# tjysdsg/speech-recognition

Measured on AMD Instinct MI355X. Metric: frame-state loglik/s + utterances/s Viterbi decode, higher is better.
Workload: dtype f64; 1 GPU; configs[1]: 10-digit HMM, 5 states/digit, 8-mix GMM, 39-dim, 10000 utterances/GPU (999364 frames on rank 0), isolated-word decode; states=50, mixtures=8, dim=39, parallelism=utterance-sharded x1, batches_in_flight=2, process_group=single

## Files before the change

speech-recognition_amd/csrc/gh_loglik_mfma.hip:

```cpp
#include "gh_internal.h"
#include "gh_wave.h"

namespace {

typedef double v4d __attribute__((ext_vector_type(4)));
typedef float v4f __attribute__((ext_vector_type(4)));

struct gh_loglik_blk { int64_t n0; int32_t nrows, t0, t1, pad; };

template <typename T> struct Acc;
template <> struct Acc<double> {
    typedef v4d type;
    static __device__ __forceinline__ v4d mfma(double a, double b, v4d c) {
        return __builtin_amdgcn_mfma_f64_16x16x4f64(a, b, c, 0, 0, 0);
    }
};
template <> struct Acc<float> {
    typedef v4f type;
    static __device__ __forceinline__ v4f mfma(float a, float b, v4f c) {
        return __builtin_amdgcn_mfma_f32_16x16x4f32(a, b, c, 0, 0, 0);
    }
};

struct Fp64Tables {
    double exp2[128];
    double inv[128];
    double nlog[128];
};

template <typename T> struct Dom;
template <> struct Dom<double> {
    static constexpr double inv_k = 1.0 / GH_LSE_SCALE64, off = GH_LSE_OFF64, off_test = GH_LSE_OFF64 * 0.1;
};
template <> struct Dom<float> {
    static constexpr float inv_k = (float)(1.0 / GH_LSE_SCALE32), off = GH_LSE_OFF32, off_test = GH_LSE_OFF32 * 0.1f;
};

struct LseK {
    double e3 = 2.6466421444330968834e-08;
    double l4 = -46.166241308446829036, l3 = 61.554988411262438714;
    double l2 = -92.332482616893658071, l1 = 184.66496523378731614;
    __device__ __forceinline__ void pin() {
        asm volatile("" : "+v"(e3), "+v"(l4), "+v"(l3), "+v"(l2), "+v"(l1));
    }
};

__device__ __forceinline__ double logs(double s, const double* __restrict__ tab, const LseK& k) {
    const double* __restrict__ inv = tab + 128;
    const double* __restrict__ nlog = tab + 256;
    const double m = __builtin_amdgcn_frexp_mant(s);
    const int e = __builtin_amdgcn_frexp_exp(s);
    const int j = (__double2hiint(m) >> 13) & 127;
    const double rho = fma(m, inv[j], -1.0);
    double p = fma(rho, 36.932993046757463228, k.l4);
    p = fma(p, rho, k.l3);
    p = fma(p, rho, k.l2);
    p = fma(p, rho, k.l1);
    return fma(p, rho, nlog[j]) + (double)(e << 7);
}
__device__ __forceinline__ float logs(float s, const double*, const LseK&) { return __builtin_amdgcn_logf(s); }

template <int W> __device__ __forceinline__ void swap_rows(unsigned v, unsigned& a, unsigned& b) {
    if (W == 16) {
        auto r = __builtin_amdgcn_permlane16_swap(v, v, false, false);
        a = r[0]; b = r[1];
    } else {
        auto r = __builtin_amdgcn_permlane32_swap(v, v, false, false);
        a = r[0]; b = r[1];
    }
}
template <int W> __device__ __forceinline__ void pair_of(float v, float& a, float& b) {
    unsigned x, y;
    swap_rows<W>(__float_as_uint(v), x, y);
    a = __uint_as_float(x); b = __uint_as_float(y);
}
template <int W> __device__ __forceinline__ void pair_of(double v, double& a, double& b) {
    unsigned xl, yl, xh, yh;
    swap_rows<W>((unsigned)__double2loint(v), xl, yl);
    swap_rows<W>((unsigned)__double2hiint(v), xh, yh);
    a = __hiloint2double((int)xh, (int)xl); b = __hiloint2double((int)yh, (int)yl);
}
template <typename T, int W> __device__ __forceinline__ T pair_max(T v) { T a, b; pair_of<W>(v, a, b); return vmax(a, b); }
template <typename T, int W> __device__ __forceinline__ T pair_sum(T v) { T a, b; pair_of<W>(v, a, b); return a + b; }
__device__ __forceinline__ void pair_split(float v0, float v1, float& a, float& b) {
    auto r = __builtin_amdgcn_permlane16_swap(__float_as_uint(v0), __float_as_uint(v1), false, false);
    a = __uint_as_float(r[0]); b = __uint_as_float(r[1]);
}
__device__ __forceinline__ void pair_split(double v0, double v1, double& a, double& b) {
    auto lo = __builtin_amdgcn_permlane16_swap((unsigned)__double2loint(v0), (unsigned)__double2loint(v1), false, false);
    auto hi = __builtin_amdgcn_permlane16_swap((unsigned)__double2hiint(v0), (unsigned)__double2hiint(v1), false, false);
    a = __hiloint2double((int)hi[0], (int)lo[0]); b = __hiloint2double((int)hi[1], (int)lo[1]);
}
template <typename T> __device__ __forceinline__ T pair_sum_split(T v0, T v1) { T a, b; pair_split(v0, v1, a, b); return a + b; }
template <typename T> __device__ __forceinline__ T pair_max_split(T v0, T v1) { T a, b; pair_split(v0, v1, a, b); return vmax(a, b); }

template <typename T> __device__ __forceinline__ T nll_of(T mx, T sm, const double* tab, T inf_below, const LseK& k) {
    const T v = (mx + logs(sm, tab, k)) * -Dom<T>::inv_k;
    return (mx < inf_below) ? T(INFINITY) : v;
}

template <typename T, typename V> __device__ __forceinline__ T lane_max(const V& a) { return vmax(vmax(a[0], a[1]), vmax(a[2], a[3])); }
template <typename T, typename V> __device__ __forceinline__ T lane_terms(const V& a, T m, const double* tab, const LseK& k) {
    return (exp2s(a[0] - m, tab, k.e3) + exp2s(a[1] - m, tab, k.e3)) + (exp2s(a[2] - m, tab, k.e3) + exp2s(a[3] - m, tab, k.e3));
}
template <typename T, typename V>
__device__ __forceinline__ void tile_lse(const V& a, int width, T& mx, T& sm, const double* tab, const LseK& k) {
    T m = lane_max<T, V>(a);
    if (width >= 2) m = pair_max<T, 16>(m);
    if (width >= 4) m = pair_max<T, 32>(m);
    T e = lane_terms<T, V>(a, m, tab, k);
    if (width >= 2) e = pair_sum<T, 16>(e);
    if (width >= 4) e = pair_sum<T, 32>(e);
    mx = m;
    sm = e;
}

__device__ __forceinline__ float exp2s_fe(double y) { return __builtin_amdgcn_exp2f((float)y * 0.0078125f); }
template <int W> __device__ __forceinline__ float pair_sum_f(float v) { float a, b; pair_of<W>(v, a, b); return a + b; }
template <typename V>
__device__ __forceinline__ void tile_lse_fe(const V& a, int width, double& mx, float& sm) {
    double m = vmax(vmax(a[0], a[1]), vmax(a[2], a[3]));
    if (width >= 2) m = pair_max<double, 16>(m);
    if (width >= 4) m = pair_max<double, 32>(m);
    float e = (exp2s_fe(a[0] - m) + exp2s_fe(a[1] - m)) + (exp2s_fe(a[2] - m) + exp2s_fe(a[3] - m));
    if (width >= 2) e = pair_sum_f<16>(e);
    if (width >= 4) e = pair_sum_f<32>(e);
    mx = m;
    sm = e;
}
__device__ __forceinline__ double nll_of_fe(double mx, float sm, double inf_below) {
    const double v = (mx + (double)(128.0f * __builtin_amdgcn_logf(sm))) * -Dom<double>::inv_k;
    return (mx < inf_below) ? (double)INFINITY : v;
}

template <typename T> using global_ptr = const T __attribute__((address_space(1)))*;
template <typename T> __device__ __forceinline__ global_ptr<T> uniform_ptr(const T* p) {
    uint32_t lo = (uint32_t)reinterpret_cast<uintptr_t>(p), hi = (uint32_t)(reinterpret_cast<uintptr_t>(p) >> 32);
    asm("" : "+s"(lo), "+s"(hi));
    return (global_ptr<T>)reinterpret_cast<const T*>(((uintptr_t)hi << 32) | lo);
}

template <typename T, typename V, int MP, bool FE = false>
__device__ __forceinline__ void tile_epilogue(const V& acc0, const V& acc1, int t, int f, int q, int S, int RS,
                                              int chunk_s0, int tiles_per_state, T* lds, T* dummy,
                                              const double* tab, T (&run_mx)[2], T (&run_sm)[2], T inf_below, const LseK& k) {
    T* orow0 = lds + f * RS - chunk_s0;
    T* orow1 = orow0 + 16 * RS;
    if (MP == 1) {
        const int s = 16 * t + 4 * q;
#pragma unroll
        for (int c = 0; c < 2; ++c) {
            const V& acc = c ? acc1 : acc0;
            T* orow = c ? orow1 : orow0;
#pragma unroll
            for (int r = 0; r < 4; ++r)
                *((s + r < S) ? orow + s + r : dummy) = (acc[r] < inf_below) ? T(INFINITY) : acc[r] * -Dom<T>::inv_k;
        }
    } else if (MP == 2) {
        const int s = 8 * t + 2 * q;
#pragma unroll
        for (int c = 0; c < 2; ++c) {
            const V& acc = c ? acc1 : acc0;
            T* orow = c ? orow1 : orow0;
#pragma unroll
            for (int h = 0; h < 2; ++h) {
                const T x0 = acc[2 * h], x1 = acc[2 * h + 1];
                const T m = vmax(x0, x1);
                const T e = exp2s(x0 - m, tab, k.e3) + exp2s(x1 - m, tab, k.e3);
                *((s + h < S) ? orow + s + h : dummy) = nll_of<T>(m, e, tab, inf_below, k);
            }
        }
#ifdef GH_MF_NOEPI
    } else if (MP <= 16) {
        const int s = (16 / MP) * t + q / (MP / 4);
        *(((q & (MP / 4 - 1)) == 0 && s < S) ? orow0 + s : dummy) = -((acc0[0] + acc0[1]) + (acc0[2] + acc0[3]));
        *(((q & (MP / 4 - 1)) == 0 && s < S) ? orow1 + s : dummy) = -((acc1[0] + acc1[1]) + (acc1[2] + acc1[3]));
#endif
    } else if (FE && MP == 4) {
        if constexpr (FE) {
            double mx; float sm;
            const int s = 4 * t + q;
            tile_lse_fe<V>(acc0, 1, mx, sm);
            *((s < S) ? orow0 + s : dummy) = nll_of_fe(mx, sm, inf_below);
            tile_lse_fe<V>(acc1, 1, mx, sm);
            *((s < S) ? orow1 + s : dummy) = nll_of_fe(mx, sm, inf_below);
        }
    } else if (FE && MP <= 16) {
        if constexpr (FE) {
            constexpr int width = MP / 4;
            double mx0, mx1; float sm0, sm1;
            tile_lse_fe<V>(acc0, width, mx0, sm0);
            tile_lse_fe<V>(acc1, width, mx1, sm1);
            const bool odd = q & 1;
            const int s = (16 / MP) * t + q / width;
            const double v = nll_of_fe(odd ? mx1 : mx0, odd ? sm1 : sm0, inf_below);
            *(((q & (width - 1)) < 2 && s < S) ? (odd ? orow1 : orow0) + s : dummy) = v;
        }
    } else if (FE) {
        if constexpr (FE) {
            const bool last = (t + 1) % tiles_per_state == 0;
            const int s = t / tiles_per_state;
#pragma unroll
            for (int c = 0; c < 2; ++c) {
                double mx; float smf;
                tile_lse_fe<V>(c ? acc1 : acc0, 4, mx, smf);
                const double d = run_mx[c] - mx;
                const float e = exp2s_fe((d > 0.0) ? -d : d);
                const float rs = (float)run_sm[c];
                run_sm[c] = (double)((d > 0.0) ? fmaf(smf, e, rs) : fmaf(rs, e, smf));
                run_mx[c] = (d > 0.0) ? run_mx[c] : mx;
            }
            const bool odd = q & 1;
            const double v = nll_of_fe(odd ? run_mx[1] : run_mx[0], (float)(odd ? run_sm[1] : run_sm[0]), inf_below);
            *((last && q < 2 && s < S) ? (odd ? orow1 : orow0) + s : dummy) = v;
#pragma unroll
            for (int c = 0; c < 2; ++c) {
                run_mx[c] = last ? Dom<T>::off : run_mx[c];
                run_sm[c] = last ? T(0) : run_sm[c];
            }
        }
    } else if (MP == 4) {
        T mx, sm;
        const int s = 4 * t + q;
        tile_lse<T, V>(acc0, 1, mx, sm, tab, k);
        *((s < S) ? orow0 + s : dummy) = nll_of<T>(mx, sm, tab, inf_below, k);
        tile_lse<T, V>(acc1, 1, mx, sm, tab, k);
        *((s < S) ? orow1 + s : dummy) = nll_of<T>(mx, sm, tab, inf_below, k);
    } else if (MP <= 16) {
        constexpr int width = MP / 4;
        T mxs = pair_max_split(lane_max<T, V>(acc0), lane_max<T, V>(acc1));
        if (width >= 4) mxs = pair_max<T, 32>(mxs);
        T mx0, mx1;
        pair_of<16>(mxs, mx0, mx1);
        T sm = pair_sum_split(lane_terms<T, V>(acc0, mx0, tab, k), lane_terms<T, V>(acc1, mx1, tab, k));
        if (width >= 4) sm = pair_sum<T, 32>(sm);
        const bool odd = q & 1;
        const int s = (16 / MP) * t + q / width;
        const T v = nll_of<T>(mxs, sm, tab, inf_below, k);
        *(((q & (width - 1)) < 2 && s < S) ? (odd ? orow1 : orow0) + s : dummy) = v;
    } else {
        const bool last = (t + 1) % tiles_per_state == 0;
        const int s = t / tiles_per_state;
#pragma unroll
        for (int c = 0; c < 2; ++c) {
            T mx, sm;
            tile_lse<T, V>(c ? acc1 : acc0, 4, mx, sm, tab, k);
            const T d = run_mx[c] - mx;
            const T e = exp2s((d > T(0)) ? -d : d, tab, k.e3);
            run_sm[c] = (d > T(0)) ? fma(sm, e, run_sm[c]) : fma(run_sm[c], e, sm);
            run_mx[c] = (d > T(0)) ? run_mx[c] : mx;
        }
        const bool odd = q & 1;
        const T v = nll_of<T>(odd ? run_mx[1] : run_mx[0], odd ? run_sm[1] : run_sm[0], tab, inf_below, k);
        *((last && q < 2 && s < S) ? (odd ? orow1 : orow0) + s : dummy) = v;
#pragma unroll
        for (int c = 0; c < 2; ++c) {
            run_mx[c] = last ? Dom<T>::off : run_mx[c];
            run_sm[c] = last ? T(0) : run_sm[c];
        }
    }
}

#ifndef GH_MF_SGB
#define GH_MF_SGB 0
#endif
template <typename T, int KS, int MP, bool MULTI, bool FE = false>
__global__ __launch_bounds__(64, (sizeof(T) == 4 ? 3 : 1)) void loglik_mfma_kernel(const T* __restrict__ X, int64_t N, int D,
                                                         const T* __restrict__ Apk, const T* __restrict__ Cpk,
                                                         int n_tiles, int S, int M_pad, int chunk_tiles,
                                                         const double* __restrict__ tables, int tab_off,
                                                         T* __restrict__ out, int bpw,
                                                         const gh_loglik_blk* __restrict__ blk_tab, int64_t n_blk,
                                                         const T* __restrict__ cen, T inf_below) {
    typedef typename Acc<T>::type V;
#ifndef GH_MF_RING32
#define GH_MF_RING32 2
#endif
#ifndef GH_MF_RING64
#define GH_MF_RING64 1
#endif
    constexpr int R = KS / (sizeof(T) == 4 ? GH_MF_RING32 : GH_MF_RING64);
    extern __shared__ __attribute__((aligned(16))) unsigned char smem_raw[];
    T* lds = reinterpret_cast<T*>(smem_raw);
    const int lane = threadIdx.x;
    const int f = lane & 15, q = lane >> 4;
    const int64_t n_blocks = (N + 31) / 32;
    int64_t n0 = (int64_t)blockIdx.x * (MULTI ? bpw : 1) * 32;
#ifdef GH_MF_TIMING
    long long tk[5], tw[2];
    tk[0] = clock64(); tw[0] = wall_clock64();
#endif
    int nrows = 0;
    const bool subset = MULTI && blk_tab != nullptr;
    const int64_t kb0 = (int64_t)blockIdx.x * (MULTI ? bpw : 1);
    int t_lo = subset ? blk_tab[kb0].t0 : 0, t_hi = n_tiles, nxt_t0 = 0;
    double* tab = reinterpret_cast<double*>(smem_raw + tab_off);
    if (sizeof(T) == 8 && MP != 1) {
        double tr[6];
#pragma unroll
        for (int it = 0; it < 6; ++it) tr[it] = tables[lane + 64 * it];
#pragma unroll
        for (int it = 0; it < 6; ++it) tab[lane + 64 * it] = tr[it];
    }
    auto stage_frames = [&]() {
        const int nelem = nrows * D;
        const T* src = X + n0 * D;
        T xr[KS];
#pragma unroll
        for (int it = 0; it < KS; ++it) {
            const int i = lane + 64 * it;
            xr[it] = (i < nelem) ? src[i] : T(0);
        }
#pragma unroll
        for (int it = 0; it < KS; ++it) {
            const int i = lane + 64 * it;
            if (i < nelem) lds[i] = xr[it];
        }
        __syncthreads();
    };
    constexpr int KQ = KS / 2;
    T b[2][KS];
    T cen_r[KQ];
#pragma unroll
    for (int j = 0; j < KQ; ++j) cen_r[j] = (sizeof(T) == 4 && cen) ? cen[4 * j + q] : T(0);
    auto build_b = [&]() {
#pragma unroll
        for (int c = 0; c < 2; ++c) {
            const int row = 16 * c + f;
#pragma unroll
            for (int j = 0; j < KQ; ++j) {
                const int d = 4 * j + q;
                T v = (row < nrows && d < D) ? lds[row * D + d] : T(0);
                if (sizeof(T) == 4) v = (row < nrows && d < D) ? v - cen_r[j] : T(0);
                b[c][j] = v * v;
                b[c][KQ + j] = v;
            }
        }
        __syncthreads();
    };

    const int tiles_per_state = (MP <= 16) ? 1 : M_pad / 16;
    const int SC = (MP <= 16) ? chunk_tiles * (16 / (MP <= 16 ? MP : 16)) : chunk_tiles / tiles_per_state;
    const int RS = (S <= SC) ? S : SC;
    T* dummy = lds + 32 * RS + lane;
    T run_mx[2] = {Dom<T>::off, Dom<T>::off}, run_sm[2] = {T(0), T(0)};
    LseK lse_k;
    if (sizeof(T) == 8 && !MULTI && !FE && MP != 1) lse_k.pin();
    int chunk_s0 = 0;
    int subset_cnt = 0;

    T ring[R];
#pragma unroll
    for (int j = 0; j < R; ++j) ring[j] = Apk[((int64_t)t_lo * KS + j) * 64 + lane];
    V c_a, c_b, p0, p1;
#pragma unroll
    for (int r = 0; r < 4; ++r) c_a[r] = Cpk[t_lo * 16 + 4 * q + r];

    auto mfma_tile = [&](int t, V& acc0, V& acc1, const V& c_use, V& c_load) {
        const int tn = (!MULTI || t + 1 < t_hi) ? t + 1 : nxt_t0;
        const global_ptr<T> cp = uniform_ptr(Cpk + (unsigned)(tn * 16));
#pragma unroll
        for (int r = 0; r < 4; ++r) c_load[r] = cp[4 * q + r];
        constexpr int WIN = 4096 / (64 * (int)sizeof(T)), NW = (KS + WIN - 1) / WIN;
        global_ptr<T> a_cur[NW], a_nxt[NW];
#pragma unroll
        for (int w = 0; w < NW; ++w) {
            a_cur[w] = uniform_ptr(Apk + (unsigned)(t * (KS * 64) + w * (WIN * 64)));
            a_nxt[w] = uniform_ptr(Apk + (unsigned)(tn * (KS * 64) + w * (WIN * 64)));
        }
#pragma unroll
        for (int ks = 0; ks < KS; ++ks) {
            const T a = ring[ks % R];
#ifdef GH_MF_NOMFMA
            if (ks == 0) { acc0 = c_use; acc1 = c_use; }
            if (ks % 8 == 0) { acc0[ks % 4] += a * b[0][ks]; acc1[ks % 4] += a * b[1][ks]; }
            else asm volatile("" :: "v"(a));
#else
            acc0 = Acc<T>::mfma(a, b[0][ks], ks == 0 ? c_use : acc0);
            acc1 = Acc<T>::mfma(a, b[1][ks], ks == 0 ? c_use : acc1);
#endif
#ifndef GH_MF_NOLOAD
            ring[ks % R] = (ks + R < KS) ? a_cur[(ks + R) / WIN][((ks + R) % WIN) * 64 + lane]
                                         : a_nxt[(ks + R - KS) / WIN][((ks + R - KS) % WIN) * 64 + lane];
#endif
        }
    };
    auto flush = [&]() {
        const int cnt = subset ? subset_cnt : ((chunk_s0 + SC < S) ? chunk_s0 + SC : S) - chunk_s0;
        __syncthreads();
        if (cnt == S && !subset) {
            typedef T V16 __attribute__((ext_vector_type(16 / sizeof(T))));
            constexpr int VE = 16 / sizeof(T);
            T* dst = out + n0 * S;
            const int total = nrows * S;
            const int nvec = total / VE;
#pragma unroll 4
            for (int i = lane; i < nvec; i += 64)
                reinterpret_cast<V16*>(dst)[i] = reinterpret_cast<const V16*>(lds)[i];
            for (int i = nvec * VE + lane; i < total; i += 64) dst[i] = lds[i];
        } else if (cnt > 0) {
            const int total = nrows * cnt;
            for (int i = lane; i < total; i += 64) {
                const int r = i / cnt, j = i - r * cnt;
                out[(n0 + r) * S + chunk_s0 + j] = lds[r * RS + j];
            }
        }
        __syncthreads();
        chunk_s0 += SC;
    };

    const int nb = MULTI ? bpw : 1;
    int64_t staged_n0 = -1;
    for (int ib = 0; ib < nb; ++ib, n0 += 32) {
        if (subset) {
            const int64_t k = kb0 + ib;
            if (k >= n_blk) break;
            const gh_loglik_blk bd = blk_tab[k];
            n0 = bd.n0; nrows = bd.nrows; t_lo = bd.t0; t_hi = bd.t1;
            nxt_t0 = (ib + 1 < nb && k + 1 < n_blk) ? blk_tab[k + 1].t0 : bd.t0;
        } else {
            if (MULTI && n0 >= N) break;
            nrows = (int)((N - n0 < 32) ? (N - n0) : 32);
        }
        if (!(subset && ib > 0 && n0 == staged_n0)) {
#ifdef GH_MF_PRIO
            __builtin_amdgcn_s_setprio(3);
#endif
            stage_frames();
            build_b();
#ifdef GH_MF_PRIO
            __builtin_amdgcn_s_setprio(0);
#endif
            staged_n0 = n0;
        }
        chunk_s0 = (MP <= 16) ? t_lo * (16 / (MP <= 16 ? MP : 16)) : t_lo / tiles_per_state;
        if (subset) {
            const int s_end = (MP <= 16) ? t_hi * (16 / (MP <= 16 ? MP : 16)) : t_hi / tiles_per_state;
            subset_cnt = ((s_end < S) ? s_end : S) - chunk_s0;
        }
#ifdef GH_MF_TIMING
        tk[1] = clock64();
        tk[2] = tk[1];
#endif
        auto epi = [&](const V& e0, const V& e1, int t) {
            tile_epilogue<T, V, MP, FE>(e0, e1, t, f, q, S, RS, chunk_s0, tiles_per_state, lds, dummy, tab, run_mx, run_sm, inf_below, lse_k);
#pragma unroll
            for (int i = 0; i < (GH_MF_SGB ? 2 * KS : 0); ++i) {
                __builtin_amdgcn_sched_group_barrier(0x008, 1, 0);
                __builtin_amdgcn_sched_group_barrier(0x002, sizeof(T) == 8 ? 5 : 3, 0);
            }
            if (!subset && (t + 1) % chunk_tiles == 0 && t + 1 < n_tiles) flush();
        };
        V r0, r1;
        const int tb = MULTI ? t_lo : 0, te = MULTI ? t_hi : n_tiles;
        mfma_tile(tb, p0, p1, c_a, c_b);
        if (sizeof(T) == 8) {
            int t = tb + 1;
            for (; t + 1 < te; t += 2) {
                mfma_tile(t, r0, r1, c_b, c_a);
                epi(p0, p1, t - 1);
                mfma_tile(t + 1, p0, p1, c_a, c_b);
                epi(r0, r1, t);
            }
            if (t < te) {
                mfma_tile(t, r0, r1, c_b, c_a);
                epi(p0, p1, t - 1);
                epi(r0, r1, t);
            } else {
                epi(p0, p1, te - 1);
                if (MULTI) c_a = c_b;
            }
        } else {
            for (int t = tb + 1; t < te; ++t) {
                mfma_tile(t, r0, r1, c_b, c_a);
                epi(p0, p1, t - 1);
                p0 = r0;
                p1 = r1;
                c_b = c_a;
            }
            epi(p0, p1, te - 1);
            if (MULTI) c_a = c_b;
        }
#ifdef GH_MF_TIMING
        tk[3] = clock64();
#endif
        flush();
#ifdef GH_MF_TIMING
        tk[4] = clock64(); tw[1] = wall_clock64();
        if (lane == 0 && S >= 8) {
            T* o = out + n0 * S;
            for (int i = 0; i < 5; ++i) o[i] = (T)(double)(tk[i] - tk[0]);
            o[5] = (T)(double)(tw[0] & 0xffffffffffll); o[6] = (T)(double)(tw[1] - tw[0]);
            o[7] = (T)(double)__builtin_amdgcn_s_getreg((4 << 0) | (0 << 6) | (31 << 11));
        }
#endif
    }
}

static void chunk_shape(const gh_gmm* g, int* chunk_tiles_out, int* SC_out) {
    const int M_pad = g->M_pad, n_tiles = g->n_tiles, S = g->S;
    int chunk_tiles;
    if (M_pad <= 16) {
        const int spt = 16 / M_pad;
        chunk_tiles = (S <= 64) ? n_tiles : std::max(1, 64 / spt);
    } else {
        const int tps = M_pad / 16;
        chunk_tiles = (S <= 64) ? n_tiles : 64 * tps;
    }
    *chunk_tiles_out = chunk_tiles;
    *SC_out = (M_pad <= 16) ? chunk_tiles * (16 / M_pad) : chunk_tiles / (M_pad / 16);
}

static int build_blk_table(const gh_gmm* g, const gh_batch* b, int SC, const int32_t* st_lo, const int32_t* st_hi,
                           const int64_t* rng_off, std::vector<gh_loglik_blk>& tabv, int* max_tiles_out,
                           const uint8_t* include = nullptr) {
    const int M_pad = g->M_pad, S = g->S;
    int max_tiles = 1;
    std::vector<std::pair<int, int>> runs;
    for (int64_t u = 0; u < b->U; ++u) {
        if (include && !include[u]) continue;
        runs.clear();
        const int64_t r0 = rng_off ? rng_off[u] : u, r1 = rng_off ? rng_off[u + 1] : u + 1;
        for (int64_t r = r0; r < r1; ++r) {
            const int lo = st_lo[r], hi = st_hi[r];
            if (lo < 0 || hi > S || lo >= hi) { gh_set_error("gh_loglik_subset: utterance %lld has state range [%d, %d)", (long long)u, lo, hi); return GH_ERR_INVALID; }
            int t0, t1;
            if (M_pad <= 16) { const int spt = 16 / M_pad; t0 = lo / spt; t1 = (hi + spt - 1) / spt; }
            else { const int tps = M_pad / 16; t0 = lo * tps; t1 = hi * tps; }
            runs.push_back({t0, t1});
        }
        std::sort(runs.begin(), runs.end());
        size_t w = 0;
        for (size_t i = 0; i < runs.size(); ++i) {
            if (w > 0 && runs[i].first <= runs[w - 1].second) runs[w - 1].second = std::max(runs[w - 1].second, runs[i].second);
            else runs[w++] = runs[i];
        }
        runs.resize(w);
        for (const auto& tr : runs) {
            const int t0 = tr.first, t1 = tr.second;
            const int span = (M_pad <= 16) ? (t1 - t0) * (16 / M_pad) : (t1 - t0) / (M_pad / 16);
            if (span > SC) return 1;
            max_tiles = std::max(max_tiles, t1 - t0);
        }
        for (int64_t f = b->offsets[u]; f < b->offsets[u + 1]; f += 32)
            for (const auto& tr : runs)
                tabv.push_back(gh_loglik_blk{f, (int32_t)std::min<int64_t>(32, b->offsets[u + 1] - f), tr.first, tr.second, 0});
    }
    *max_tiles_out = max_tiles;
    return GH_OK;
}

template <typename T>
int launch_mfma_t(gh_ctx* ctx, const gh_gmm* g, gh_batch* b, const T* Apk, const T* Cpk, const int32_t* st_lo,
                  const int32_t* st_hi, const T* cen, const int64_t* rng_off, const gh_loglik_plan* plan) {
    const int64_t N = b->N;
    if (N == 0) return GH_OK;
    const int KS = g->KP / 2;
    const int M_pad = g->M_pad, n_tiles = g->n_tiles, S = g->S;
    int chunk_tiles, SC;
    chunk_shape(g, &chunk_tiles, &SC);
    size_t lds = ((size_t)32 * std::max(std::min(SC, S), g->D) + 64) * sizeof(T);
    lds = (lds + 15) & ~size_t(15);
    const int tab_off = (int)lds;
    if (sizeof(T) == 8 && M_pad != 1) lds += 384 * sizeof(double);
    const double* tables = ctx->d_fp64_tables;
    const T inf_below = (ctx->compat & 1) ? (T)(-745.1332191019412 * (sizeof(T) == 8 ? GH_LSE_SCALE64 : GH_LSE_SCALE32)) : Dom<T>::off_test;
    gh_loglik_blk* d_blk = nullptr;
    int64_t n_blk = 0;
    int max_tiles = n_tiles;
    if (plan) {
        d_blk = static_cast<gh_loglik_blk*>(plan->d_blk);
        n_blk = plan->n_blk;
        max_tiles = plan->max_tiles;
        if (n_blk == 0) return GH_OK;
    } else if (st_lo) {
        std::vector<gh_loglik_blk> tabv;
        int rc = build_blk_table(g, b, SC, st_lo, st_hi, rng_off, tabv, &max_tiles);
        if (rc) return rc;
        n_blk = (int64_t)tabv.size();
        if (n_blk == 0) return GH_OK;
        void* base;
        rc = gh_scratch(ctx, tabv.size() * sizeof(gh_loglik_blk), &base);
        if (rc) return rc;
        d_blk = static_cast<gh_loglik_blk*>(base);
        GH_HIP(hipMemcpyAsync(d_blk, tabv.data(), tabv.size() * sizeof(gh_loglik_blk), hipMemcpyHostToDevice, ctx->stream));
        GH_HIP(hipStreamSynchronize(ctx->stream));
    }
    const bool subset = plan || st_lo;
    const int64_t n_blocks = subset ? n_blk : (N + 31) / 32;
    const int per_block = std::max(1, max_tiles * KS * 2);
    int bpw = (int)std::max<int64_t>(1, std::min<int64_t>(8, (512 + per_block - 1) / per_block));
    if (const char* e = getenv("GMMHMM_LOGLIK_BPW")) bpw = std::max(1, std::min(16, atoi(e)));
    if (subset) bpw = std::max(bpw, 2);
    const unsigned grid = (unsigned)((n_blocks + bpw - 1) / bpw);
    const T* X = static_cast<const T*>(b->feats);
    T* out = static_cast<T*>(b->nll);
    const bool fe = sizeof(T) == 8 && (ctx->compat & 2) && M_pad >= 4;
#define GH_MF_LAUNCH(ks, mp)                                                                                             \
    do {                                                                                                                 \
        if (fe && sizeof(T) == 8 && mp >= 4) {                                                                           \
            if (bpw > 1)                                                                                                 \
                hipLaunchKernelGGL((loglik_mfma_kernel<T, ks, mp, true, (sizeof(T) == 8 && mp >= 4)>), dim3(grid), dim3(64), lds, ctx->stream, X, N, g->D, \
                                   Apk, Cpk, n_tiles, S, M_pad, chunk_tiles, tables, tab_off, out, bpw, d_blk, n_blk, cen, inf_below); \
            else                                                                                                         \
                hipLaunchKernelGGL((loglik_mfma_kernel<T, ks, mp, false, (sizeof(T) == 8 && mp >= 4)>), dim3(grid), dim3(64), lds, ctx->stream, X, N, g->D, \
                                   Apk, Cpk, n_tiles, S, M_pad, chunk_tiles, tables, tab_off, out, bpw, d_blk, n_blk, cen, inf_below); \
        } else if (bpw > 1)                                                                                                     \
            hipLaunchKernelGGL((loglik_mfma_kernel<T, ks, mp, true>), dim3(grid), dim3(64), lds, ctx->stream, X, N, g->D, \
                               Apk, Cpk, n_tiles, S, M_pad, chunk_tiles, tables, tab_off, out, bpw, d_blk, n_blk, cen, inf_below); \
        else                                                                                                             \
            hipLaunchKernelGGL((loglik_mfma_kernel<T, ks, mp, false>), dim3(grid), dim3(64), lds, ctx->stream, X, N, g->D, \
                               Apk, Cpk, n_tiles, S, M_pad, chunk_tiles, tables, tab_off, out, bpw, d_blk, n_blk, cen, inf_below); \
    } while (0)
#define GH_MF_CASE(ks)                                   \
    case ks:                                             \
        switch (M_pad) {                                 \
            case 1: GH_MF_LAUNCH(ks, 1); break;          \
            case 2: GH_MF_LAUNCH(ks, 2); break;          \
            case 4: GH_MF_LAUNCH(ks, 4); break;          \
            case 8: GH_MF_LAUNCH(ks, 8); break;          \
            case 16: GH_MF_LAUNCH(ks, 16); break;        \
            default: GH_MF_LAUNCH(ks, 32); break;        \
        }                                                \
        break;
    switch (KS) {
        GH_MF_CASE(2)
        GH_MF_CASE(4)
        GH_MF_CASE(8)
        GH_MF_CASE(12)
        GH_MF_CASE(20)
        GH_MF_CASE(24)
        GH_MF_CASE(32)
        default:
            return 1;
    }
#undef GH_MF_CASE
#undef GH_MF_LAUNCH
    GH_HIP(hipGetLastError());
    return GH_OK;
}

}

int gh_launch_loglik_mfma(gh_ctx* ctx, const gh_gmm* g, gh_batch* b, const int32_t* st_lo, const int32_t* st_hi,
                          const int64_t* rng_off, const gh_loglik_plan* plan) {
    if (!g->dApk64) return 1;
    b->nll_serial = g->serial;
    if (b->dtype == GH_F64) return launch_mfma_t<double>(ctx, g, b, g->dApk64, g->dCpk64, st_lo, st_hi, nullptr, rng_off, plan);
    return launch_mfma_t<float>(ctx, g, b, g->dApk32, g->dCpk32, st_lo, st_hi, g->dCen32, rng_off, plan);
}

int gh_loglik_plan_build(gh_ctx* ctx, const gh_gmm* g, const gh_batch* b, const int32_t* st_lo, const int32_t* st_hi,
                         const int64_t* rng_off, gh_loglik_plan* out, const uint8_t* include) {
    out->d_blk = nullptr; out->n_blk = 0; out->max_tiles = 1;
    if (!g->dApk64) return 1;
    const int KS = g->KP / 2;
    if (KS != 2 && KS != 4 && KS != 8 && KS != 12 && KS != 20 && KS != 24 && KS != 32) return 1;
    int chunk_tiles, SC;
    chunk_shape(g, &chunk_tiles, &SC);
    std::vector<gh_loglik_blk> tabv;
    int rc = build_blk_table(g, b, SC, st_lo, st_hi, rng_off, tabv, &out->max_tiles, include);
    if (rc) return rc;
    out->n_blk = (int64_t)tabv.size();
    if (tabv.empty()) return GH_OK;
    GH_HIP(hipMalloc(&out->d_blk, tabv.size() * sizeof(gh_loglik_blk)));
    GH_HIP(hipMemcpy(out->d_blk, tabv.data(), tabv.size() * sizeof(gh_loglik_blk), hipMemcpyHostToDevice));
    return GH_OK;
}

void gh_loglik_plan_free(gh_loglik_plan* p) {
    if (p && p->d_blk) hipFree(p->d_blk);
    if (p) { p->d_blk = nullptr; p->n_blk = 0; }
}
```

Measured before the change: 41.39 billion frame-state loglik/s.

## Split tail-wave loglik blocks across state-tile pieces to fill idle CUs

Computes resident workgroup slots via the occupancy API and, when the last wave of 32-frame blocks only partially fills the GPU, splits each of those remaining blocks into up to 4 workgroups that each handle a disjoint range of state tiles. Each piece writes only its own columns. This targets the tail-wave imbalance where a few workgroups run alone on a mostly idle device. The cost is redundant frame staging in each piece, an occupancy query cached per kernel, and several env knobs for tuning.

```diff
diff --git a/speech-recognition_amd/csrc/gh_loglik_mfma.hip b/speech-recognition_amd/csrc/gh_loglik_mfma.hip
--- a/speech-recognition_amd/csrc/gh_loglik_mfma.hip
+++ b/speech-recognition_amd/csrc/gh_loglik_mfma.hip
@@ -1,5 +1,8 @@
 #include "gh_internal.h"
 #include "gh_wave.h"
+#include <map>
+#include <mutex>
+#include <utility>
 
 namespace {
 
@@ -271,7 +274,7 @@
                                                          const double* __restrict__ tables, int tab_off,
                                                          T* __restrict__ out, int bpw,
                                                          const gh_loglik_blk* __restrict__ blk_tab, int64_t n_blk,
-                                                         const T* __restrict__ cen, T inf_below) {
+                                                         const T* __restrict__ cen, T inf_below, int tail_first, int tail_p) {
     typedef typename Acc<T>::type V;
 #ifndef GH_MF_RING32
 #define GH_MF_RING32 2
@@ -284,8 +287,18 @@
     T* lds = reinterpret_cast<T*>(smem_raw);
     const int lane = threadIdx.x;
     const int f = lane & 15, q = lane >> 4;
-    const int64_t n_blocks = (N + 31) / 32;
-    int64_t n0 = (int64_t)blockIdx.x * (MULTI ? bpw : 1) * 32;
+    const int tiles_per_state = (MP <= 16) ? 1 : M_pad / 16;
+    int64_t blk = blockIdx.x;
+    int piece_lo = 0, piece_hi = n_tiles;
+    const bool piece = !MULTI && tail_p > 1 && (int)blockIdx.x >= tail_first;
+    if (piece) {
+        const int j = (int)blockIdx.x - tail_first, k = j / tail_p, i = j - k * tail_p;
+        const int units = n_tiles / tiles_per_state;
+        blk = tail_first + k;
+        piece_lo = (int)((int64_t)i * units / tail_p) * tiles_per_state;
+        piece_hi = (int)((int64_t)(i + 1) * units / tail_p) * tiles_per_state;
+    }
+    int64_t n0 = (MULTI ? (int64_t)blockIdx.x * bpw : blk) * 32;
 #ifdef GH_MF_TIMING
     long long tk[5], tw[2];
     tk[0] = clock64(); tw[0] = wall_clock64();
@@ -293,7 +306,7 @@
     int nrows = 0;
     const bool subset = MULTI && blk_tab != nullptr;
     const int64_t kb0 = (int64_t)blockIdx.x * (MULTI ? bpw : 1);
-    int t_lo = subset ? blk_tab[kb0].t0 : 0, t_hi = n_tiles, nxt_t0 = 0;
+    int t_lo = subset ? blk_tab[kb0].t0 : piece_lo, t_hi = piece_hi, nxt_t0 = 0;
     double* tab = reinterpret_cast<double*>(smem_raw + tab_off);
     if (sizeof(T) == 8 && MP != 1) {
         double tr[6];
@@ -339,7 +352,6 @@
         __syncthreads();
     };
 
-    const int tiles_per_state = (MP <= 16) ? 1 : M_pad / 16;
     const int SC = (MP <= 16) ? chunk_tiles * (16 / (MP <= 16 ? MP : 16)) : chunk_tiles / tiles_per_state;
     const int RS = (S <= SC) ? S : SC;
     T* dummy = lds + 32 * RS + lane;
@@ -383,6 +395,13 @@
             ring[ks % R] = (ks + R < KS) ? a_cur[(ks + R) / WIN][((ks + R) % WIN) * 64 + lane]
                                          : a_nxt[(ks + R - KS) / WIN][((ks + R - KS) % WIN) * 64 + lane];
 #endif
+        }
+    };
+    auto write_cols = [&](int cnt) {
+        const int total = nrows * cnt;
+        for (int i = lane; i < total; i += 64) {
+            const int r = i / cnt, j = i - r * cnt;
+            out[(n0 + r) * S + chunk_s0 + j] = lds[r * RS + j];
         }
     };
     auto flush = [&]() {
@@ -399,11 +418,7 @@
                 reinterpret_cast<V16*>(dst)[i] = reinterpret_cast<const V16*>(lds)[i];
             for (int i = nvec * VE + lane; i < total; i += 64) dst[i] = lds[i];
         } else if (cnt > 0) {
-            const int total = nrows * cnt;
-            for (int i = lane; i < total; i += 64) {
-                const int r = i / cnt, j = i - r * cnt;
-                out[(n0 + r) * S + chunk_s0 + j] = lds[r * RS + j];
-            }
+            write_cols(cnt);
         }
         __syncthreads();
         chunk_s0 += SC;
@@ -434,7 +449,7 @@
             staged_n0 = n0;
         }
         chunk_s0 = (MP <= 16) ? t_lo * (16 / (MP <= 16 ? MP : 16)) : t_lo / tiles_per_state;
-        if (subset) {
+        if (subset || piece) {
             const int s_end = (MP <= 16) ? t_hi * (16 / (MP <= 16 ? MP : 16)) : t_hi / tiles_per_state;
             subset_cnt = ((s_end < S) ? s_end : S) - chunk_s0;
         }
@@ -449,10 +464,10 @@
                 __builtin_amdgcn_sched_group_barrier(0x008, 1, 0);
                 __builtin_amdgcn_sched_group_barrier(0x002, sizeof(T) == 8 ? 5 : 3, 0);
             }
-            if (!subset && (t + 1) % chunk_tiles == 0 && t + 1 < n_tiles) flush();
+            if (!subset && (t + 1) % chunk_tiles == 0 && t + 1 < t_hi) flush();
         };
         V r0, r1;
-        const int tb = MULTI ? t_lo : 0, te = MULTI ? t_hi : n_tiles;
+        const int tb = t_lo, te = t_hi;
         mfma_tile(tb, p0, p1, c_a, c_b);
         if (sizeof(T) == 8) {
             int t = tb + 1;
@@ -484,7 +499,12 @@
 #ifdef GH_MF_TIMING
         tk[3] = clock64();
 #endif
-        flush();
+        if (!MULTI && piece) {
+            __syncthreads();
+            write_cols(subset_cnt);
+        } else {
+            flush();
+        }
 #ifdef GH_MF_TIMING
         tk[4] = clock64(); tw[1] = wall_clock64();
         if (lane == 0 && S >= 8) {
@@ -550,6 +570,36 @@
     return GH_OK;
 }
 
+static int resident_wgs(const void* fn, size_t lds) {
+    static std::mutex mu;
+    static std::map<std::pair<const void*, size_t>, int> cache;
+    std::lock_guard<std::mutex> lock(mu);
+    auto it = cache.find({fn, lds});
+    if (it != cache.end()) return it->second;
+    int n = 0;
+    if (hipOccupancyMaxActiveBlocksPerMultiprocessor(&n, fn, 64, lds) != hipSuccess) { (void)hipGetLastError(); n = 0; }
+    cache[{fn, lds}] = n;
+    return n;
+}
+
+static void tail_plan(const gh_ctx* ctx, const void* fn, size_t lds, int64_t n_blocks, int units, unsigned* grid,
+                      int* tail_first, int* tail_p) {
+    if (const char* e = getenv("GMMHMM_LOGLIK_TAIL")) if (atoi(e) == 0) return;
+    const int64_t slots = (int64_t)resident_wgs(fn, lds) * ctx->n_cu;
+    if (slots <= 0) return;
+    int64_t r = n_blocks % slots;
+    if (const char* e = getenv("GMMHMM_LOGLIK_TAIL_BLOCKS")) r = std::max<int64_t>(0, std::min<int64_t>(n_blocks, atoll(e)));
+    if (r <= 0) return;
+    const int P = (int)std::min<int64_t>(std::min<int64_t>(4, units), slots / r);
+    if (P < 2 || n_blocks - r + r * P > 0x7fffffff) return;
+    *tail_first = (int)(n_blocks - r);
+    *tail_p = P;
+    *grid = (unsigned)(n_blocks - r + r * P);
+    if (const char* e = getenv("GMMHMM_HOST_TRACE")) if (atoi(e))
+        fprintf(stderr, "[gh_loglik] tail: %lld of %lld blocks in %d pieces each (%lld resident workgroups)\n", (long long)r,
+                (long long)n_blocks, P, (long long)slots);
+}
+
 template <typename T>
 int launch_mfma_t(gh_ctx* ctx, const gh_gmm* g, gh_batch* b, const T* Apk, const T* Cpk, const int32_t* st_lo,
                   const int32_t* st_hi, const T* cen, const int64_t* rng_off, const gh_loglik_plan* plan) {
@@ -563,6 +613,7 @@
     lds = (lds + 15) & ~size_t(15);
     const int tab_off = (int)lds;
     if (sizeof(T) == 8 && M_pad != 1) lds += 384 * sizeof(double);
+    if (const char* e = getenv("GMMHMM_LOGLIK_LDS_PAD")) lds = std::min<size_t>(65536, lds + (size_t)std::max(0, atoi(e)));
     const double* tables = ctx->d_fp64_tables;
     const T inf_below = (ctx->compat & 1) ? (T)(-745.1332191019412 * (sizeof(T) == 8 ? GH_LSE_SCALE64 : GH_LSE_SCALE32)) : Dom<T>::off_test;
     gh_loglik_blk* d_blk = nullptr;
@@ -596,21 +647,27 @@
     const T* X = static_cast<const T*>(b->feats);
     T* out = static_cast<T*>(b->nll);
     const bool fe = sizeof(T) == 8 && (ctx->compat & 2) && M_pad >= 4;
+    const bool tail_ok = !subset && bpw == 1 && S <= SC;
+    const int tail_units = (M_pad <= 16) ? n_tiles : n_tiles / (M_pad / 16);
+#define GH_MF_ONE(kern)                                                                                                  \
+    do {                                                                                                                 \
+        unsigned grid1 = grid;                                                                                           \
+        int tail_first = 0, tail_p = 1;                                                                                  \
+        if (tail_ok) tail_plan(ctx, reinterpret_cast<const void*>(&kern), lds, n_blocks, tail_units, &grid1, &tail_first, &tail_p); \
+        hipLaunchKernelGGL((kern), dim3(grid1), dim3(64), lds, ctx->stream, X, N, g->D, Apk, Cpk, n_tiles, S, M_pad,     \
+                           chunk_tiles, tables, tab_off, out, bpw, d_blk, n_blk, cen, inf_below, tail_first, tail_p);    \
+    } while (0)
 #define GH_MF_LAUNCH(ks, mp)                                                                                             \
     do {                                                                                                                 \
         if (fe && sizeof(T) == 8 && mp >= 4) {                                                                           \
             if (bpw > 1)                                                                                                 \
-                hipLaunchKernelGGL((loglik_mfma_kernel<T, ks, mp, true, (sizeof(T) == 8 && mp >= 4)>), dim3(grid), dim3(64), lds, ctx->stream, X, N, g->D, \
-                                   Apk, Cpk, n_tiles, S, M_pad, chunk_tiles, tables, tab_off, out, bpw, d_blk, n_blk, cen, inf_below); \
+                GH_MF_ONE((loglik_mfma_kernel<T, ks, mp, true, (sizeof(T) == 8 && mp >= 4)>));                            \
             else                                                                                                         \
-                hipLaunchKernelGGL((loglik_mfma_kernel<T, ks, mp, false, (sizeof(T) == 8 && mp >= 4)>), dim3(grid), dim3(64), lds, ctx->stream, X, N, g->D, \
-                                   Apk, Cpk, n_tiles, S, M_pad, chunk_tiles, tables, tab_off, out, bpw, d_blk, n_blk, cen, inf_below); \
-        } else if (bpw > 1)                                                                                                     \
-            hipLaunchKernelGGL((loglik_mfma_kernel<T, ks, mp, true>), dim3(grid), dim3(64), lds, ctx->stream, X, N, g->D, \
-                               Apk, Cpk, n_tiles, S, M_pad, chunk_tiles, tables, tab_off, out, bpw, d_blk, n_blk, cen, inf_below); \
+                GH_MF_ONE((loglik_mfma_kernel<T, ks, mp, false, (sizeof(T) == 8 && mp >= 4)>));                           \
+        } else if (bpw > 1)                                                                                              \
+            GH_MF_ONE((loglik_mfma_kernel<T, ks, mp, true>));                                                            \
         else                                                                                                             \
-            hipLaunchKernelGGL((loglik_mfma_kernel<T, ks, mp, false>), dim3(grid), dim3(64), lds, ctx->stream, X, N, g->D, \
-                               Apk, Cpk, n_tiles, S, M_pad, chunk_tiles, tables, tab_off, out, bpw, d_blk, n_blk, cen, inf_below); \
+            GH_MF_ONE((loglik_mfma_kernel<T, ks, mp, false>));                                                           \
     } while (0)
 #define GH_MF_CASE(ks)                                   \
     case ks:                                             \
@@ -636,6 +693,7 @@
     }
 #undef GH_MF_CASE
 #undef GH_MF_LAUNCH
+#undef GH_MF_ONE
     GH_HIP(hipGetLastError());
     return GH_OK;
 }
```

Result: no change. 41.74 billion frame-state loglik/s, median of 6 (+0.8%).
